# MinJunKang/DualPixelFace

Measured on AMD Instinct MI355X. Metric: train samples/sec, StereoDPNet 1024x1536 DP pair, higher is better.
Workload: dtype f32

## Files before the change

### dualpixelface_amd/csrc/conv_api.hip

```cpp
#include "conv_internal.h"
#include <cstdlib>

namespace {

int g_operand_bf16 = 0;
int g_f32_x9 = -1;
int g_h3_guard = 1;

int clamp_x9(int v) { return v < 0 ? 0 : (v > 2 ? 2 : v); }

int out_dim(int I, int k, int s, int p, int d) { return (I + 2 * p - (d * (k - 1) + 1)) / s + 1; }

DpfConvDesc forward_desc(int N, int C, int ID, int IH, int IW, int K, int kd, int kh, int kw, int sd, int sh, int sw, int pd, int ph, int pw, int dd,
                         int dh, int dw) {
  return {N, C, K, K, 0, ID, IH, IW, out_dim(ID, kd, sd, pd, dd), out_dim(IH, kh, sh, ph, dh), out_dim(IW, kw, sw, pw, dw),
          kd, kh, kw, sd, sh, sw, pd, ph, pw, dd, dh, dw,  0,  K, C,  0,  0};
}
DpfConvDesc transposed_desc(int N, int C, int ID, int IH, int IW, int K, int Ktot, int OD, int OH, int OW, int kd, int kh, int kw, int sd, int sh,
                            int sw, int pd, int ph, int pw, int dd, int dh, int dw, int accumulate) {
  return {N, C, K, Ktot, 0, ID, IH, IW, OD, OH, OW, kd, kh, kw, sd, sh, sw, pd, ph, pw, dd, dh, dw,  1, C, Ktot,  1, accumulate};
}

bool bad_args(const void* a, const void* b, const void* c, int N, int C, int K) { return !a || !b || !c || N <= 0 || C <= 0 || K <= 0; }

int conv_dispatch(const float* x, const float* w, const float* bias, float* out, float* ws, const DpfConvDesc& d, DpfConvStats* stats, hipStream_t st) {
  const int T = d.kd * d.kh * d.kw;
  const bool plain = !stats && !d.accumulate;
  if (!plain && d.K > 128) return DPF_ERR_UNSUPPORTED;
  if (T > DPF_CONV_MAXT)
    return !stats && dpf_wide_eligible(T, d.kd, d.kh, d.kw, d.sd, d.sh, d.sw, d.pd, d.dd, d.dh, d.dw) ? dpf_wide_conv(x, w, bias, out, d, st)
                                                                                                        : DPF_ERR_UNSUPPORTED;
  if (T < 1) return DPF_ERR_UNSUPPORTED;
  for (int k0 = 0; k0 < d.K; k0 += 128) {
    DpfConvDesc s = d;
    s.k0 = k0;
    s.K = d.K - k0 < 128 ? d.K - k0 : 128;
    int rc = DPF_ERR_UNSUPPORTED;
    if (plain && T == 1) rc = dpf_pointwise_conv(x, w, bias, out, s, st);
    if (rc == DPF_ERR_UNSUPPORTED) rc = dpf_igemm2_conv(x, w, bias, out, ws, s, st, stats);
    if (rc == DPF_ERR_UNSUPPORTED && plain) rc = dpf_gen1_conv(x, w, bias, out, ws, s, st);
    if (rc != DPF_OK) return rc;
  }
  return DPF_OK;
}

int wgrad_dispatch(const float* g, const float* x, float* dw, float* ws, long long ws_floats, const DpfWgradDesc& d, int accumulate, hipStream_t st) {
  const int T = d.kd * d.kh * d.kw;
  for (int k0 = 0; k0 < d.K; k0 += 128) {
    DpfWgradDesc s = d;
    s.k0 = k0;
    s.K = d.K - k0 < 128 ? d.K - k0 : 128;
    float* dwk = dw + (long long)k0 * d.C * T;
    int rc = DPF_ERR_UNSUPPORTED;
    if (ws && T == 1) rc = dpf_pointwise_wgrad(g, x, dwk, ws, ws_floats, s, accumulate, st);
    if (rc == DPF_ERR_UNSUPPORTED && ws && T > DPF_CONV_MAXT) rc = dpf_wide_wgrad(g, x, dwk, ws, ws_floats, s, accumulate, st);
    if (rc == DPF_ERR_UNSUPPORTED && ws) rc = dpf_wgrad2(g, x, dwk, ws, ws_floats, s, accumulate, st);
    if (rc == DPF_ERR_UNSUPPORTED) {
      if (!accumulate && hipMemsetAsync(dwk, 0, sizeof(float) * (size_t)s.K * d.C * T, st) != hipSuccess) return DPF_ERR_LAUNCH;
      rc = dpf_gen1_wgrad(g, x, dwk, s, st);
    }
    if (rc != DPF_OK) return rc;
  }
  return DPF_OK;
}

}

const ConvEnv& conv_env() {
  static const ConvEnv env = [] {
    auto num = [](const char* v, int unset) { return v ? atoi(v) : unset; };
    ConvEnv e;
    e.f32_x9 = clamp_x9(num(getenv("DPF_F32_X9"), 2));
    e.igemm2 = num(getenv("DPF_IGEMM2"), 1);
    e.igemm2_tr2 = num(getenv("DPF_IGEMM2_TR2"), 1);
    e.igemm2_1x1 = num(getenv("DPF_IGEMM2_1x1"), 1);
    e.igemm3 = num(getenv("DPF_IGEMM3"), 1);
    e.igemm3_cc = num(getenv("DPF_IGEMM3_CC"), 0);
    e.igemm3_sh = num(getenv("DPF_IGEMM3_SH"), -1);
    e.igemm3_rstep = num(getenv("DPF_IGEMM3_RSTEP"), 1);
    e.igemm3_bf = num(getenv("DPF_IGEMM3_BF"), 1);
    e.g2_pz = num(getenv("DPF_G2_PZ"), 0);
    e.g2_vec_store = num(getenv("DPF_G2_VEC_STORE"), 1);
    e.wgrad2 = num(getenv("DPF_WGRAD2"), 1);
    e.w2_sw1 = num(getenv("DPF_W2_SW1"), 1);
    e.w2_rstep = num(getenv("DPF_W2_RSTEP"), 1);
    e.pointwise = num(getenv("DPF_POINTWISE"), 1);
    return e;
  }();
  return env;
}

int dpf_conv_operand_bf16() { return g_operand_bf16; }
int dpf_conv_f32_x9() { return g_f32_x9 < 0 ? conv_env().f32_x9 : g_f32_x9; }
int dpf_h3_range_guard() { return g_h3_guard; }

extern "C" {

int dpf_set_conv_operand_precision(int bf16) {
  g_operand_bf16 = bf16 ? 1 : 0;
  return DPF_OK;
}
int dpf_get_conv_operand_precision(void) { return g_operand_bf16; }
int dpf_set_f32_matrix_path(int split_bf16) {
  g_f32_x9 = clamp_x9(split_bf16);
  return DPF_OK;
}
int dpf_get_f32_matrix_path(void) { return dpf_conv_f32_x9(); }
int dpf_debug_set_range_guard(int on) {
  g_h3_guard = on ? 1 : 0;
  return DPF_OK;
}

long long dpf_conv_workspace_floats(int T, int reduce, int outc) {
  const long long a = (long long)T * reduce * (((outc + 31) / 32) * 32), b = dpf_igemm2_workspace_floats(T, reduce, outc);
  return a > b ? a : b;
}

int dpf_conv_forward(const float* x, const float* w, const float* bias, float* out, float* ws, int N, int C, int ID, int IH, int IW,
                     int K, int kd, int kh, int kw, int sd, int sh, int sw, int pd, int ph, int pw, int dd, int dh, int dw,
                     void* stream) {
  dpf_clear_error();
  if (bad_args(x, w, out, N, C, K) || !ws) return DPF_ERR_INVALID_ARG;
  const DpfConvDesc d = forward_desc(N, C, ID, IH, IW, K, kd, kh, kw, sd, sh, sw, pd, ph, pw, dd, dh, dw);
  if (d.OD <= 0 || d.OH <= 0 || d.OW <= 0) return DPF_ERR_INVALID_ARG;
  return conv_dispatch(x, w, bias, out, ws, d, nullptr, (hipStream_t)stream);
}

long long dpf_conv_stats_slab_doubles(int N, int K, int OD, int OH, int OW) {
  return 2LL * K * ((long long)N * OD * dpf_div_up(OH, 8) * dpf_div_up(OW, 32) + 64);
// ... 41 lines not shown
```

### dualpixelface_amd/csrc/conv_igemm2.hip

```cpp
#include "conv_internal.h"
#include <type_traits>

namespace {

constexpr int MAXT = 27;
constexpr int NLD = 8;
constexpr int ZPAGE = 16;

struct G2P {
  int N, C, K, Ktot, k0;
  int ID, IH, IW, OD, OH, OW;
  int sxd, sxh, sxw;
  int e0d, e0h, e0w;
  int ext_d, ext_h;
  int pz, thp, thp_shift, odt;
  int planeStride;
  int RS, SR;
  int colshift;
  int rpc, chanStride;
  int nseg;
  int nwseg;
  int T;
  int tilesH, tilesW;
  int ntiles, cpx;
// ... 344 lines not shown
        for (int cp = 0; cp < CC / 2; ++cp)
  #pragma unroll
          for (int m = 0; m < MT; ++m)
  #pragma unroll
            for (int t = 0; t < NT; ++t) acc[m][t] = __builtin_amdgcn_mfma_f32_32x32x2f32(a[cp][m], bb[cp][t], acc[m][t], 0, 0, 0);
      };
      auto touch = [&](const float (&a)[CC / 2][MT], const float (&bb)[CC / 2][NT]) {
  #pragma unroll
        for (int cp = 0; cp < CC / 2; ++cp) {
  #pragma unroll
          for (int m = 0; m < MT; ++m) asm volatile("" ::"v"(a[cp][m]));
  #pragma unroll
          for (int t = 0; t < NT; ++t) asm volatile("" ::"v"(bb[cp][t]));
        }
        asm volatile("" ::: "memory");
      };
      load_ops(aA, bA);
      for (int slot = 0; slot + 1 < nv; slot += 2) {
        touch(aA, bA);
        load_ops(aB, bB);
        __builtin_amdgcn_sched_barrier(6);
        mfmas(aA, bA);
        __builtin_amdgcn_sched_barrier(0);
        touch(aB, bB);
        load_ops(aA, bA);
        __builtin_amdgcn_sched_barrier(6);
        mfmas(aB, bB);
        __builtin_amdgcn_sched_barrier(0);
      }
      if (nv & 1) mfmas(aA, bA);
    }
    __builtin_amdgcn_sched_barrier(0);
    __syncthreads();
    if (single && chunk + 1 < p.nchunks) {
      issue(chunk + 1, 0);
      __syncthreads();
    }
  }

  g2_epilogue<MT, NT>(acc, p, bias, out, smem, tile_id, n, qd, q0h, q0w, wave, l31, hh, tid);
}



typedef unsigned u32x4 __attribute__((ext_vector_type(4)));
typedef __bf16 bf16x8 __attribute__((ext_vector_type(8)));
typedef _Float16 f16x8 __attribute__((ext_vector_type(8)));

__device__ __forceinline__ void split_pair(float x, float y, unsigned& h, unsigned& m, unsigned& l) { dpf_split_pair(x, y, h, m, l); }

constexpr int X9_FIRST = DPF_X9_FIRST;
constexpr int X9_NP = 9 - X9_FIRST;

template <int CC, int NC> struct X9 {
  static constexpr int NU = CC == 4 ? 2 : 1;
  static constexpr int PB = 2 * NC * CC;
  static constexpr int TPG = 16 / CC;
  static constexpr int PD = PB / 4;
};

#ifdef DPF_STAMPS
__device__ unsigned long long g_x9_passes[4];
__device__ unsigned long long g_x9_stamps[8 * 16384];
#define X9_STAMP(slot, val) if (tid == 0 && blockIdx.x < 16384) g_x9_stamps[blockIdx.x * 8 + (slot)] = (val);
#define X9_COUNT(slot) if (tid == 0) atomicAdd(&g_x9_passes[slot], 1ull);
#else
#define X9_STAMP(slot, val)
#define X9_COUNT(slot)
#endif

template <int MT, int NT, int CC, bool SH, int NC = 3>
__global__ __launch_bounds__(256, 2) void igemm3_x9_kernel(const float* __restrict__ x, const unsigned short* __restrict__ wpk,
                                                           const float* __restrict__ bias, float* __restrict__ out, G2P p) {
  extern __shared__ __attribute__((aligned(16))) float smem[];
  static_assert(NT == 2 || NT == 4, "position rows are processed in pairs");
  constexpr int KT = 32 * MT;
  constexpr int NU = X9<CC, NC>::NU, PB = X9<CC, NC>::PB, TPG = X9<CC, NC>::TPG, PD = X9<CC, NC>::PD;
  constexpr int NPROD = NC == 3 ? X9_NP : (NC == 2 ? 3 : 1);
  constexpr int SPV = NC == 3 ? 9 : (NC == 2 ? 6 : 1);
  constexpr int NPS = NT / 2;
  constexpr int NSL = NU * 4;
  const int tid = threadIdx.x;
  const int lane = tid & 63;
  const int wave = __builtin_amdgcn_readfirstlane(tid >> 6);
  const int l31 = lane & 31;
  const int hh = lane >> 5;

  int b = (blockIdx.x & 7) * p.cpx + (blockIdx.x >> 3);
  if (b >= p.ntiles) return;
  X9_STAMP(0, __builtin_readcyclecounter()) X9_STAMP(4, __builtin_amdgcn_s_memrealtime())
  const int tile_id = b;
  const int qd = (b % p.odt) * p.pz; b /= p.odt;
  const int tw = b % p.tilesW; b /= p.tilesW;
  const int th = b % p.tilesH;
  const int n = b / p.tilesH;
  const int q0h = (th / p.rstep) * (p.thp * p.rstep) + th % p.rstep, q0w = tw * 32;
  const int i0d = qd + p.e0d, i0h = q0h + p.e0h;
  const int a0 = q0w + p.e0w - p.colshift;

  const int TG = (p.T + TPG - 1) / TPG;
  const int patchBytes = PB * p.rpc * p.RS;
  const int wBytes = TG * NC * MT * 1024;
  char* s_patch = reinterpret_cast<char*>(smem);
  char* s_w = s_patch + patchBytes;
  int* s_tab = reinterpret_cast<int*>(s_w + (SH ? 2 : 1) * wBytes);
  int* s_red = s_tab + 32;
  int Ex = DPF_H3_EMIN;
  int Erun = DPF_H3_EMIN;
  float scx = 0.f;
  unsigned tbC = 0, tbN = 0;
  unsigned kminL = 0xffffffffu;
  const long long x_chan = (long long)p.ID * p.IH * p.IW;
  const float* xn = x + (long long)n * p.C * x_chan;
  const int nunits = p.rpc * p.SR;

  if (tid < 32) s_tab[tid] = tid < 28 ? PB * p.tapoff[tid] : 0;

  int goff[NU], loff[NU];
#pragma unroll
  for (int j = 0; j < NU; ++j) {
    const unsigned f = tid + 256 * j;
    const unsigned row = (f * p.mSR) >> 20;
    const int seg = f - row * p.SR;
    const unsigned pl = (row * p.mEH) >> 20;
    const int rr = row - pl * p.ext_h;
    const int id = i0d + (int)pl, ih = i0h + rr * p.rstep, iw = a0 + 4 * seg;
    const bool ok = (int)f < nunits && id >= 0 && id < p.ID && ih >= 0 && ih < p.IH && iw >= 0 && iw < p.IW;
    goff[j] = ok ? (int)(((long long)id * p.IH + ih) * p.IW + iw) : -1;
    loff[j] = (int)f < nunits ? PB * ((int)row * p.RS + 4 * seg) : -1;
  }

  f32x4 pv[NU][CC];
  unsigned sp[NU][4][PD];
  auto prefetch = [&](int chunk) {
    const float* xc = xn + (long long)chunk * CC * x_chan;
    const int crem = p.C - chunk * CC;
#pragma unroll
    for (int j = 0; j < NU; ++j)
#pragma unroll
      for (int ch = 0; ch < CC; ++ch) {
        f32x4 v = {0.f, 0.f, 0.f, 0.f};
        if (goff[j] >= 0 && ch < crem) v = *reinterpret_cast<const f32x4*>(xc + (long long)ch * x_chan + goff[j]);
        pv[j][ch] = v;
      }
  };
  auto issue_w = [&](int chunk, int buf) {
    const char* wc = reinterpret_cast<const char*>(wpk) + (long long)chunk * wBytes;
    char* dst = s_w + buf * wBytes;
    const int nws = wBytes >> 4;
    for (int f0 = wave * 64; f0 < nws; f0 += 256) {
      const int f = f0 + lane;
      if (f < nws) glds16(reinterpret_cast<const float*>(wc + f * 16), reinterpret_cast<float*>(dst + f0 * 16));
    }
  };
  auto split_slice = [&](int sl) {
    const int j = sl >> 2, ps = sl & 3;
#pragma unroll
    for (int k = 0; k < CC / 2; ++k) {
      if constexpr (NC == 3) split_pair(pv[j][2 * k][ps], pv[j][2 * k + 1][ps], sp[j][ps][k], sp[j][ps][CC / 2 + k], sp[j][ps][CC + k]);
      else if constexpr (NC == 2) dpf_split_pair_h(pv[j][2 * k][ps] * scx, pv[j][2 * k + 1][ps] * scx, sp[j][ps][k], sp[j][ps][CC / 2 + k]);
      else sp[j][ps][k] = pk_bf16(pv[j][2 * k][ps], pv[j][2 * k + 1][ps]);
    }
  };
  auto pos_max = [&](int j, int ps) {
    float mp = __builtin_fabsf(pv[j][0][ps]);
#pragma unroll
    for (int ch = 1; ch < CC; ++ch) mp = __builtin_fmaxf(mp, __builtin_fabsf(pv[j][ch][ps]));
    return mp;
  };
  auto post_exp = [&]() {
    float pm[NU][4];
#pragma unroll
    for (int j = 0; j < NU; ++j) {
#pragma unroll
      for (int ps = 0; ps < 4; ++ps) pm[j][ps] = __builtin_fmaxf(__builtin_fabsf(pv[j][0][ps]), __builtin_fabsf(pv[j][1][ps]));
#pragma unroll
      for (int ch = 2; ch < CC; ch += 2)
#pragma unroll
        for (int ps = 0; ps < 4; ++ps) pm[j][ps] = __builtin_fmaxf(__builtin_fmaxf(pm[j][ps], __builtin_fabsf(pv[j][ch][ps])), __builtin_fabsf(pv[j][ch + 1][ps]));
    }
    float m = 0.f;
    kminL = 0xffffffffu;
// ... 14 lines not shown
    return e > 254 ? 254 : (e < DPF_H3_EMIN ? DPF_H3_EMIN : e);
  };
  auto tb_of = [&](int e) {
    return (unsigned)(e < 1 ? 1 : (e > 254 ? 254 : e)) << 23;
  };
  int Enext = Ex;
  auto next_chunk_scale = [&]() {
    const int e = read_exp();
    Erun = e > Erun ? e : Erun;
    const int lo = Erun - DPF_H3_MAXDROP;
    Enext = (e > Ex || (e < Ex - 3 && e > DPF_H3_EMIN)) ? (e > lo ? e : lo) : Ex;
    scx = dpf_h3_scale(Enext);
    tbN = p.guard ? tb_of(Enext - DPF_H3_RANGE) : 0u;
  };
  auto next_residual_scale = [&](int pass_next) {
    const int e = read_exp();
    const int lo = Erun - DPF_H3_MAXDROP;
    const int en = Ex + e - 141;
    Enext = en > lo ? en : lo;
    if (Enext > Ex) Enext = Ex;
    scx = __builtin_bit_cast(float, (unsigned)(127 + Ex - Enext) << 23);
    tbN = pass_next < DPF_H3_MAXPASS ? tb_of(Enext - DPF_H3_RANGE + 141 - Ex) : 0u;
  };
  auto lane_defers = [&](int par) {
    const bool fl = tbN != 0u && kminL < tbN - 1u;
    if (fl) s_red[8 + par] = 1;
    return __builtin_amdgcn_ballot_w64(fl) != 0ull;
  };
  auto split_masked = [&]() {
#pragma unroll
    for (int j = 0; j < NU; ++j)
#pragma unroll
      for (int ps = 0; ps < 4; ++ps) {
        const float ml = __builtin_bit_cast(unsigned, pos_max(j, ps)) >= tbN ? scx : 0.f;
#pragma unroll
        for (int k = 0; k < CC / 2; ++k) dpf_split_pair_h(pv[j][2 * k][ps] * ml, pv[j][2 * k + 1][ps] * ml, sp[j][ps][k], sp[j][ps][CC / 2 + k]);
      }
  };
  auto residual_update = [&]() {
#pragma unroll
    for (int j = 0; j < NU; ++j)
#pragma unroll
      for (int ps = 0; ps < 4; ++ps) {
        const float ml = __builtin_bit_cast(unsigned, pos_max(j, ps)) >= tbC ? 0.f : scx;
#pragma unroll
        for (int ch = 0; ch < CC; ++ch) pv[j][ch][ps] *= ml;
      }
  };
  auto store_split = [&]() {
#pragma unroll
    for (int j = 0; j < NU; ++j)
      if (loff[j] >= 0) {
        u32x4* dst = reinterpret_cast<u32x4*>(s_patch + loff[j]);
#pragma unroll
        for (int i = 0; i < PD; ++i) {
          const int e = 4 * i;
          const u32x4 v = {sp[j][e / PD][e % PD], sp[j][(e + 1) / PD][(e + 1) % PD], sp[j][(e + 2) / PD][(e + 2) % PD], sp[j][(e + 3) / PD][(e + 3) % PD]};
          dst[i] = v;
        }
      }
  };

  f32x16 acc[MT][NT];
#pragma unroll
  for (int m = 0; m < MT; ++m)
#pragma unroll
    for (int t = 0; t < NT; ++t)
#pragma unroll
      for (int j = 0; j < 16; ++j) acc[m][t][j] = 0.f;
  auto rescale_acc = [&](int de) {
#pragma unroll
    for (int m = 0; m < MT; ++m)
#pragma unroll
      for (int t = 0; t < NT; ++t)
#pragma unroll
        for (int j = 0; j < 16; ++j) acc[m][t][j] = __builtin_ldexpf(acc[m][t][j], de);
  };

  int lb[NT];
#pragma unroll
  for (int t = 0; t < NT; ++t) {
    const int r = wave * NT + t, rz = r >> p.thp_shift, ry = r & (p.thp - 1);
    lb[t] = PB * (rz * p.planeStride + ry * p.RS + l31 + p.colshift);
  }

  if constexpr (NC == 2) {
    if (tid < 2) s_red[8 + tid] = 0;
  }
  if constexpr (SH) issue_w(0, 0);
  prefetch(0);
  int par = 0;
  if constexpr (SH) {
    bool wdef = false;
    if constexpr (NC == 2) {
      post_exp();
      __syncthreads();
      next_chunk_scale();
      Ex = Enext;
      wdef = lane_defers(par);
    }
#pragma unroll
    for (int sl = 0; sl < NSL; ++sl) split_slice(sl);
    if constexpr (NC == 2) {
      if (__builtin_expect(wdef, 0)) split_masked();
    }
  }

  int pass = 0;
  for (int chunk = 0; chunk < p.nchunks;) {
    if constexpr (!SH) {
      bool wdef = false;
      if (pass == 0) issue_w(chunk, 0);
      if constexpr (NC == 2) {
        post_exp();
        __syncthreads();
        if (pass == 0) next_chunk_scale(); else next_residual_scale(pass);
        wdef = lane_defers(par);
      }
#pragma unroll
      for (int sl = 0; sl < NSL; ++sl) split_slice(sl);
      if constexpr (NC == 2) {
        if (__builtin_expect(wdef, 0)) split_masked();
      }
    }
    bool more = false;
    int dflag = 0;
    if constexpr (NC == 2) {
      if constexpr (SH) {
        if (chunk > 0 || pass > 0) dflag = s_red[8 + par];
      }
      if (tid == 0) s_red[8 + (par ^ 1)] = 0;
      if (__builtin_expect(Enext != Ex, 0)) { rescale_acc(Ex - Enext); Ex = Enext; X9_COUNT(2) }
      X9_COUNT(0)
      if (pass > 0) { X9_COUNT(1) }
      tbC = tbN;
    }
// ... 526 lines not shown
}

__global__ void igemm2_pack_bf16_kernel(const float* __restrict__ w, unsigned short* __restrict__ wpk, int wA, int wB, int T, int KT, int nchunks,
                                        int mode, int k0, int K, int C) {
  const long long total = (long long)nchunks * T * 8 * KT + 2 * ZPAGE;
  for (long long i = (long long)blockIdx.x * blockDim.x + threadIdx.x; i < total; i += (long long)gridDim.x * blockDim.x) {
    float v = 0.f;
    if (i >= 2 * ZPAGE) {
      const long long e = i - 2 * ZPAGE;
      const int ii = (int)(e & 3);
      const int k = (int)((e >> 2) % KT);
      const int half = (int)((e / (4LL * KT)) & 1);
      const int t = (int)((e / (8LL * KT)) % T);
      const int chunk = (int)(e / (8LL * KT * T));
      const int c = chunk * 8 + half * 4 + ii;
      if (k < K && c < C) {
        const int a = mode == 0 ? k0 + k : c;
        const int bb = mode == 0 ? c : k0 + k;
        v = w[((long long)a * wB + bb) * T + t];
      }
    }
    wpk[i] = (unsigned short)(pk_bf16(v, 0.f) & 0xffffu);
  }
}

unsigned magic20(int d) { return (unsigned)(((1u << 20) + d - 1) / d); }

template <typename W, typename P>
struct TileLaunch {
  const float* x; const W* wpk; const float* bias; float* out; const P& p; size_t lds; long long blocks; hipStream_t st;
};

template <int MT, int NT, int CC, bool BF = false>
int launch_g2(const TileLaunch<float, G2P>& a) {
  return conv_launch<igemm2_kernel<MT, NT, CC, BF>>(dim3((unsigned)a.blocks), dim3(256), a.lds, a.st, a.x, a.wpk, a.bias, a.out, a.p);
}
template <int MT, int NT, int CC>
int launch_x9(bool sh, int NC, const TileLaunch<unsigned short, G2P>& a) {
  const dim3 grid((unsigned)a.blocks), block(256);
  switch (2 * NC + (sh ? 1 : 0)) {
    case 7: return conv_launch<igemm3_x9_kernel<MT, NT, CC, true, 3>>(grid, block, a.lds, a.st, a.x, a.wpk, a.bias, a.out, a.p);
    case 6: return conv_launch<igemm3_x9_kernel<MT, NT, CC, false, 3>>(grid, block, a.lds, a.st, a.x, a.wpk, a.bias, a.out, a.p);
    case 5: return conv_launch<igemm3_x9_kernel<MT, NT, CC, true, 2>>(grid, block, a.lds, a.st, a.x, a.wpk, a.bias, a.out, a.p);
    case 4: return conv_launch<igemm3_x9_kernel<MT, NT, CC, false, 2>>(grid, block, a.lds, a.st, a.x, a.wpk, a.bias, a.out, a.p);
    case 3: return conv_launch<igemm3_x9_kernel<MT, NT, CC, true, 1>>(grid, block, a.lds, a.st, a.x, a.wpk, a.bias, a.out, a.p);
    default: return conv_launch<igemm3_x9_kernel<MT, NT, CC, false, 1>>(grid, block, a.lds, a.st, a.x, a.wpk, a.bias, a.out, a.p);
  }
}
template <int CC, bool BF = false>
int launch_t2(const TileLaunch<float, T2P>& a) {
  return conv_launch<igemm2_tr2_kernel<CC, BF>>(dim3((unsigned)a.blocks), dim3(256), a.lds, a.st, a.x, a.wpk, a.bias, a.out, a.p);
}

int launch_x9(int MT, int NT, int CC9, bool sh, int NC, const TileLaunch<unsigned short, G2P>& a) {
  if (CC9 == 4) {
    if (MT == 1) return NT == 4 ? launch_x9<1, 4, 4>(sh, NC, a) : launch_x9<1, 2, 4>(sh, NC, a);
    return launch_x9<2, 2, 4>(sh, NC, a);
  }
  if (MT == 1) return NT == 4 ? launch_x9<1, 4, 8>(sh, NC, a) : launch_x9<1, 2, 8>(sh, NC, a);
  return launch_x9<2, 2, 8>(sh, NC, a);
}

int x9_try(const float* x, const float* w, const float* bias, float* out, float* ws, const DpfConvDesc& d, const G2P& p, int k_off, int kn, int NT,
           DpfConvStats* stats, hipStream_t st, int NC, int mt_fit = 0) {
  const ConvEnv& env = conv_env();
  constexpr int x9_min_c = 8;
  const int T = d.kd * d.kh * d.kw, MT = (kn + 31) / 32, TH = 4 * NT;
  if (!env.igemm3 || (NC >= 2 && !dpf_conv_f32_x9()) || MT > 2 || NT * MT > 4 || d.C < x9_min_c) return DPF_ERR_UNSUPPORTED;
  G2P q = p;
  q.K = kn; q.k0 = d.k0 + k_off;
  q.rstep = (env.igemm3_rstep && d.kd == 1 && d.kh > 1 && d.dh > 1) ? d.dh : 1;
  const int dhl = d.dh / q.rstep;
  int CC9 = ((T + 1) / 2) * 2 < ((T + 3) / 4) * 4 ? 8 : 4;
  if (env.igemm3_cc == 4 || env.igemm3_cc == 8) CC9 = env.igemm3_cc;
  const int NU9 = CC9 == 4 ? 2 : 1, PB9 = 2 * NC * CC9;
  auto set_pz = [&](int pz) {
    q.pz = pz; q.thp = TH / pz; q.thp_shift = 0;
    while ((1 << q.thp_shift) < q.thp) ++q.thp_shift;
    q.odt = dpf_div_up(d.OD, pz);
    q.ext_d = (pz - 1) + (d.kd - 1) * d.dd + 1;
    q.ext_h = (q.thp - 1) + (d.kh - 1) * dhl + 1;
    q.planeStride = q.ext_h * q.RS; q.SR = q.RS / 4; q.rpc = q.ext_d * q.ext_h;
    return q.rpc * q.SR;
  };
  const int TG = (T + 16 / CC9 - 1) / (16 / CC9);
  int best = 0, best_units = 1 << 30, sh = 0;
  for (int shc : {1, 0}) {
    if (best || (env.igemm3_sh >= 0 && shc != env.igemm3_sh)) continue;
    for (int pz : {1, 2, 4}) {
      if (!(pz == 1 || (d.kd > 1 && pz <= TH / 2 && pz <= d.OD))) continue;
      const int units = set_pz(pz);
      const size_t l9 = (size_t)PB9 * q.rpc * q.RS + (size_t)(shc ? 2 : 1) * TG * NC * (mt_fit > MT ? mt_fit : MT) * 1024 + 256;
      if (units <= NU9 * 256 && 2 * l9 <= 160 * 1024 && units < best_units) { best = pz; best_units = units; sh = shc; }
    }
  }
  if (!best || TG < 2) return DPF_ERR_UNSUPPORTED;
  set_pz(best);
  const size_t lds9 = (size_t)PB9 * q.rpc * q.RS + (size_t)(sh ? 2 : 1) * TG * NC * MT * 1024 + 256;
  if ((long long)NU9 * 256 * (q.SR > q.ext_h ? q.SR : q.ext_h) >= (1LL << 20)) return DPF_ERR_UNSUPPORTED;
  const int sgn = d.transposed ? -1 : 1;
  const int t0 = d.transposed ? ((d.kd - 1) * d.dd * q.ext_h + (d.kh - 1) * dhl) * q.RS + (d.kw - 1) * d.dw : 0;
  for (int u = 0; u < 28; ++u) {
    const int c = u % d.kw, b2 = (u / d.kw) % d.kh, a = u / (d.kw * d.kh);
    q.tapoff[u] = u < T ? t0 + sgn * ((a * d.dd * q.ext_h + b2 * dhl) * q.RS + c * d.dw) : 0;
  }
  q.nchunks = (d.C + CC9 - 1) / CC9;
  q.tilesH = dpf_div_up(d.OH, q.thp * q.rstep) * q.rstep;
  q.tilesW = dpf_div_up(d.OW, 32);
  q.mSR = magic20(q.SR); q.mEH = magic20(q.ext_h);
  const long long nt9 = (long long)d.N * q.odt * q.tilesH * q.tilesW;
  if (nt9 <= 0 || nt9 > 0x3fffffffLL) return DPF_ERR_INVALID_ARG;
  q.ntiles = (int)nt9;
  q.cpx = (int)((nt9 + 7) / 8);
  q.stats = nullptr;
  if (stats) {
    if (nt9 * d.K * 2 > stats->capacity_doubles) return DPF_ERR_UNSUPPORTED;
    if (k_off > 0 && stats->parts != (int)nt9) return DPF_ERR_LAUNCH;
    q.stats = stats->slab; q.statsK = d.K; q.statsk0 = k_off;
  }
  unsigned short* wp = reinterpret_cast<unsigned short*>(ws);
  const long long total = (long long)q.nchunks * TG * MT * 512;
  int* wexp = reinterpret_cast<int*>(wp + ((total * NC + 7) & ~7LL));
  q.wexp = wexp;
  q.guard = dpf_h3_range_guard();
  if (NC == 2)
    hipLaunchKernelGGL(igemm3_pack_x9h_kernel, dim3(32 * MT), dim3(256), 0, st, w, wp, d.wA, d.wB, T, TG, MT, CC9, q.nchunks, d.mode, q.k0, kn, d.C, wexp);
  else
    hipLaunchKernelGGL(igemm3_pack_x9_kernel, dim3(dpf_ew_grid(total)), dim3(256), 0, st, w, wp, d.wA, d.wB, T, TG, MT, CC9, NC, q.nchunks, d.mode, q.k0, kn,
                       d.C);
  if (dpf_check_launch() != DPF_OK) return DPF_ERR_LAUNCH;
  if (stats) stats->parts = (int)nt9;
  return launch_x9(MT, NT, CC9, sh != 0, NC, {x, wp, bias, out, q, lds9, 8LL * q.cpx, st});
}

int igemm2_tr2(const float* x, const float* w, const float* bias, float* out, float* ws, const DpfConvDesc& d, hipStream_t st) {
  if (!conv_env().igemm2_tr2) return DPF_ERR_UNSUPPORTED;
  if (d.kd != 3 || d.kh != 3 || d.kw != 3 || d.sd != 2 || d.sh != 2 || d.sw != 2 || d.pd != 1 || d.ph != 1 || d.pw != 1 || d.dd != 1 ||
      d.dh != 1 || d.dw != 1)
    return DPF_ERR_UNSUPPORTED;
  if (d.OD > 2 * d.ID || d.OH > 2 * d.IH || d.OW > 2 * d.IW) return DPF_ERR_UNSUPPORTED;
  const long long x_chan = (long long)d.ID * d.IH * d.IW;
  if (9 * x_chan >= (1LL << 30)) return DPF_ERR_UNSUPPORTED;
  const bool bf = dpf_conv_operand_bf16() != 0;
  const int CC = 8;
  T2P p{};
  p.N = d.N; p.C = d.C; p.Ktot = d.Ktot;
  p.ID = d.ID; p.IH = d.IH; p.IW = d.IW; p.OD = d.OD; p.OH = d.OH; p.OW = d.OW;
  p.RS = 36; p.SR = 9; p.rpc = 2 * 5; p.chanStride = p.rpc * p.RS;
  p.nseg = CC * p.rpc * p.SR;
  p.nwseg = bf ? 27 * 32 : 27 * CC * 32 / 4;
  p.nchunks = (d.C + CC - 1) / CC;
  p.QD = dpf_div_up(d.OD, 2);
  p.tilesH = dpf_div_up(dpf_div_up(d.OH, 2), 4);
  p.tilesW = dpf_div_up(dpf_div_up(d.OW, 2), 32);
  const long long ntiles = (long long)d.N * p.QD * p.tilesH * p.tilesW;
  if (ntiles <= 0 || ntiles > 0x3fffffffLL) return DPF_ERR_INVALID_ARG;
  p.ntiles = (int)ntiles;
  p.cpx = (int)((ntiles + 7) / 8);
  p.mSR = magic20(p.SR); p.mRPC = magic20(p.rpc); p.mEH = magic20(5);
  p.vec = conv_env().g2_vec_store;
  const size_t lds = 2 * (size_t)(CC * p.chanStride + 4 * p.nwseg) * sizeof(float);
  for (int k0 = 0; k0 < d.K; k0 += 32) {
    const int Kc = d.K - k0 < 32 ? d.K - k0 : 32;
    p.K = Kc; p.k0 = d.k0 + k0;
    const long long total = (long long)p.nchunks * 27 * CC * 32 + ZPAGE;
    if (bf)
      hipLaunchKernelGGL(igemm2_pack_bf16_kernel, dim3(dpf_ew_grid(total)), dim3(256), 0, st, w, reinterpret_cast<unsigned short*>(ws), d.wA, d.wB, 27,
                         32, p.nchunks, d.mode, p.k0, Kc, d.C);
    else
      hipLaunchKernelGGL(igemm2_pack_kernel, dim3(dpf_ew_grid(total)), dim3(256), 0, st, w, ws, d.wA, d.wB, 27, 32, CC, p.nchunks, d.mode, p.k0, Kc, d.C);
    if (dpf_check_launch() != DPF_OK) return DPF_ERR_LAUNCH;
    const TileLaunch<float, T2P> a{x, ws, bias, out, p, lds, 8LL * p.cpx, st};
    int rc;
    if (bf) rc = launch_t2<8, true>(a);
    else switch (CC) { case 2: rc = launch_t2<2>(a); break; case 4: rc = launch_t2<4>(a); break; default: rc = launch_t2<8>(a); break; }
    if (rc != DPF_OK) return rc;
  }
  return DPF_OK;
}

struct G2Plan {
  G2P p;
  int T, MT, KT;
  int NT;
  int single;
// ... 54 lines not shown
  p.accum = d.accumulate;
  p.rstep = 1;
  p.vec = conv_env().g2_vec_store && (d.OW & 3) == 0 && (reinterpret_cast<uintptr_t>(out) & 15) == 0;
  if (!d.transposed) {
    p.sxd = d.sd; p.sxh = d.sh; p.sxw = d.sw;
    p.e0d = -d.pd; p.e0h = -d.ph; p.e0w = -d.pw;
  } else {
    p.sxd = p.sxh = p.sxw = 1;
    p.e0d = d.pd - (d.kd - 1) * d.dd; p.e0h = d.ph - (d.kh - 1) * d.dh; p.e0w = d.pw - (d.kw - 1) * d.dw;
  }
  const int ext_w = 31 * p.sxw + (d.kw - 1) * d.dw + 1;
  p.colshift = ((p.e0w % 4) + 4) % 4;
  p.RS = ((p.colshift + ext_w + 3) / 4) * 4;
  const int pz_over = conv_env().g2_pz;
  auto pz_ok = [&](int pz) { return pz == 1 || (d.kd > 1 && pz <= TH / 2 && pz <= d.OD); };
  auto pz_cost = [&](int pz) {
    const int thp = TH / pz;
    return (double)((pz - 1) * p.sxd + (d.kd - 1) * d.dd + 1) * ((thp - 1) * p.sxh + (d.kh - 1) * d.dh + 1) / (double)(pz * thp);
  };
  p.pz = 1;
  for (int pz : {2, 4})
    if (pz_ok(pz) && pz_cost(pz) < pz_cost(p.pz) - 1e-9) p.pz = pz;
  if ((pz_over == 1 || pz_over == 2 || pz_over == 4) && pz_ok(pz_over)) p.pz = pz_over;
  p.thp = TH / p.pz;
  p.thp_shift = 0;
  while ((1 << p.thp_shift) < p.thp) ++p.thp_shift;
  p.odt = dpf_div_up(d.OD, p.pz);
  p.ext_d = (p.pz - 1) * p.sxd + (d.kd - 1) * d.dd + 1;
  p.ext_h = (p.thp - 1) * p.sxh + (d.kh - 1) * d.dh + 1;
  p.planeStride = p.ext_h * p.RS;
  p.SR = p.RS / 4;
  p.rpc = p.ext_d * p.ext_h;
  p.chanStride = p.rpc * p.RS;
}

void g2_tap_steps(const DpfConvDesc& d, G2P& p) {
  const int sgn = d.transposed ? -1 : 1;
  const int stepA = sgn * d.dd * p.ext_h * p.RS, stepB = sgn * d.dh * p.RS;
  p.stepC = sgn * d.dw;
  p.incB = stepB - (d.kw - 1) * p.stepC;
  p.incA = stepA - (d.kh - 1) * stepB - (d.kw - 1) * p.stepC;
  p.steps = 0;
  for (int t = 0; t < p.T; ++t) {
    const int c = t % d.kw, b = (t / d.kw) % d.kh;
    const unsigned long long code = t == p.T - 1 ? 3 : (c + 1 < d.kw ? 0 : (b + 1 < d.kh ? 1 : 2));
    p.steps |= code << (2 * t);
  }
  p.tap0 = d.transposed ? ((d.kd - 1) * d.dd * p.ext_h + (d.kh - 1) * d.dh) * p.RS + (d.kw - 1) * d.dw : 0;
}

int g2_x9_route(const float* x, const float* w, const float* bias, float* out, float* ws, const DpfConvDesc& d, const G2Plan& g, DpfConvStats* stats,
                hipStream_t st) {
  const G2P& p = g.p;
  if (!(g.T > 4 && p.sxd == 1 && p.sxh == 1 && p.sxw == 1 && (!g.bf_mode || (conv_env().igemm3_bf && !(d.K > 64 && d.kd == 1)))))
    return DPF_ERR_UNSUPPORTED;
  const int nc = g.bf_mode ? 1 : dpf_conv_f32_nc();
  if (d.K <= 64) return x9_try(x, w, bias, out, ws, d, p, 0, d.K, g.MT == 1 ? 4 : 2, stats, st, nc);
  for (int k_off = 0; k_off < d.K; k_off += 64) {
    const int rc = x9_try(x, w, bias, out, ws, d, p, k_off, d.K - k_off < 64 ? d.K - k_off : 64, 2, stats, st, nc, 2);
    if (rc == DPF_ERR_UNSUPPORTED && k_off == 0) return rc;
    if (rc != DPF_OK) return rc == DPF_ERR_UNSUPPORTED ? DPF_ERR_LAUNCH : rc;
  }
  return DPF_OK;
}

size_t g2_buf_bytes(const G2Plan& g, int cc) { return (size_t)(cc * g.p.chanStride + g.T * cc * g.KT) * sizeof(float); }
size_t g2_bf_buf_bytes(const G2Plan& g) { return (size_t)8 * g.p.chanStride * sizeof(float) + (size_t)g.T * g.KT * 16; }

bool g2_chunk(const DpfConvDesc& d, G2Plan& g) {
  constexpr int lds_target = 53 * 1024;
  const G2P& p = g.p;
  auto nseg_of = [&](int cc) { return cc * p.rpc * p.SR; };
  auto fits = [&](int cc) { return 2 * g2_buf_bytes(g, cc) <= (size_t)lds_target && nseg_of(cc) <= NLD * 256; };
  const long long ntiles_est = (long long)d.N * p.odt * dpf_div_up(d.OH, p.thp) * dpf_div_up(d.OW, 32);
  g.CC = g.bf ? 8 : (ntiles_est >= 512 && fits(2)) ? 2 : fits(8) ? 8 : fits(4) ? 4 : 2;
  return g.bf ? (nseg_of(8) <= 2 * NLD * 256 && 2 * g2_bf_buf_bytes(g) <= 160 * 1024)
              : (nseg_of(g.CC) <= NLD * 256 && 2 * g2_buf_bytes(g, g.CC) <= 160 * 1024);
}

int launch_g2(int MT, int NT, int CC, bool bf, const TileLaunch<float, G2P>& a) {
  if (bf) {
    if (NT == 4) return MT == 1 ? launch_g2<1, 4, 8, true>(a) : launch_g2<2, 4, 8, true>(a);
    switch (MT) {
      case 1: return launch_g2<1, 2, 8, true>(a);
      case 2: return launch_g2<2, 2, 8, true>(a);
      case 3: return launch_g2<3, 2, 8, true>(a);
      default: return launch_g2<4, 2, 8, true>(a);
    }
  }
  const int cc = CC == 8 ? 0 : (CC == 4 ? 1 : 2);
  switch ((NT == 4 ? (MT == 1 ? 0 : 1) : (MT < 4 ? MT + 1 : 5)) * 3 + cc) {
    case 0: return launch_g2<1, 4, 8>(a);
    case 1: return launch_g2<1, 4, 4>(a);
    case 2: return launch_g2<1, 4, 2>(a);
    case 3: return launch_g2<2, 4, 8>(a);
    case 4: return launch_g2<2, 4, 4>(a);
    case 5: return launch_g2<2, 4, 2>(a);
    case 6: return launch_g2<1, 2, 8>(a);
    case 7: return launch_g2<1, 2, 4>(a);
    case 8: return launch_g2<1, 2, 2>(a);
    case 9: return launch_g2<2, 2, 8>(a);
    case 10: return launch_g2<2, 2, 4>(a);
    case 11: return launch_g2<2, 2, 2>(a);
    case 12: return launch_g2<3, 2, 8>(a);
    case 13: return launch_g2<3, 2, 4>(a);
    case 14: return launch_g2<3, 2, 2>(a);
    case 15: return launch_g2<4, 2, 8>(a);
    case 16: return launch_g2<4, 2, 4>(a);
// ... 77 lines not shown
```

### dualpixelface_amd/csrc/conv_internal.h

```cpp
#pragma once
#include "dpf_common.h"

struct DpfConvDesc {
  int N, C, K, Ktot, k0;
  int ID, IH, IW, OD, OH, OW;
  int kd, kh, kw, sd, sh, sw, pd, ph, pw, dd, dh, dw;
  int transposed;
  int wA, wB, mode;
  int accumulate;
};

struct ConvEnv {
  int f32_x9;
  int igemm2;
  int igemm2_tr2;
  int igemm2_1x1;
  int igemm3;
  int igemm3_cc;
  int igemm3_sh;
  int igemm3_rstep;
  int igemm3_bf;
  int g2_pz;
  int g2_vec_store;
  int wgrad2;
  int w2_sw1;
  int w2_rstep;
  int pointwise;
};
const ConvEnv& conv_env();

constexpr int DPF_CONV_MAXT = 27;

int dpf_conv_operand_bf16();
int dpf_conv_f32_x9();
int dpf_h3_range_guard();
inline int dpf_conv_f32_nc() { return dpf_conv_f32_x9() == 2 ? 2 : 3; }

#ifdef __HIPCC__
template <auto Kern, typename... A>
int conv_launch(dim3 grid, dim3 block, size_t lds, hipStream_t st, A... args) {
  static size_t granted = 48 * 1024;
  if (lds > granted) {
    if (hipFuncSetAttribute((const void*)Kern, hipFuncAttributeMaxDynamicSharedMemorySize, (int)lds) != hipSuccess) return DPF_ERR_LAUNCH;
    granted = lds;
  }
  hipLaunchKernelGGL(Kern, grid, block, lds, st, args...);
  return dpf_check_launch();
}
#endif

struct DpfConvStats {
  double* slab;
  long long capacity_doubles;
  int parts;
};
int dpf_igemm2_conv(const float* x, const float* w, const float* bias, float* out, float* ws, const DpfConvDesc& d, hipStream_t st,
                    DpfConvStats* stats = nullptr);
long long dpf_igemm2_workspace_floats(int T, int reduce, int outc);
int dpf_gen1_conv(const float* x, const float* w, const float* bias, float* out, float* ws, const DpfConvDesc& d, hipStream_t st);

struct DpfWgradDesc {
  int N, C, K, Ktot, k0;
  int ID, IH, IW, QD, QH, QW;
  int kd, kh, kw, sd, sh, sw, pd, ph, pw, dd, dh, dw;
};
int dpf_wgrad2(const float* g, const float* x, float* dw, float* ws, long long ws_floats, const DpfWgradDesc& d, int accumulate, hipStream_t st);
long long dpf_wgrad2_workspace_floats(int T, int C, int K);
int dpf_gen1_wgrad(const float* g, const float* x, float* dw, const DpfWgradDesc& d, hipStream_t st);

int dpf_pointwise_conv(const float* x, const float* w, const float* bias, float* out, const DpfConvDesc& d, hipStream_t st);
int dpf_pointwise_wgrad(const float* g, const float* x, float* dw, float* ws, long long ws_floats, const DpfWgradDesc& d, int accumulate,
                        hipStream_t st);
long long dpf_pointwise_wgrad_workspace_floats(int C, int K);

// ... 75 lines not shown
```

Baseline: 27.49.

## Route stride-2 f32 convolutions through the split-precision igemm3 x9 kernel

```diff
diff --git a/dualpixelface_amd/csrc/conv_api.hip b/dualpixelface_amd/csrc/conv_api.hip
--- a/dualpixelface_amd/csrc/conv_api.hip
+++ b/dualpixelface_amd/csrc/conv_api.hip
@@ -75,6 +75,7 @@
     e.igemm2_tr2 = num(getenv("DPF_IGEMM2_TR2"), 1);
     e.igemm2_1x1 = num(getenv("DPF_IGEMM2_1x1"), 1);
     e.igemm3 = num(getenv("DPF_IGEMM3"), 1);
+    e.igemm3_s2 = e.igemm3 != 2;
     e.igemm3_cc = num(getenv("DPF_IGEMM3_CC"), 0);
     e.igemm3_sh = num(getenv("DPF_IGEMM3_SH"), -1);
     e.igemm3_rstep = num(getenv("DPF_IGEMM3_RSTEP"), 1);
diff --git a/dualpixelface_amd/csrc/conv_igemm2.hip b/dualpixelface_amd/csrc/conv_igemm2.hip
--- a/dualpixelface_amd/csrc/conv_igemm2.hip
+++ b/dualpixelface_amd/csrc/conv_igemm2.hip
@@ -420,6 +420,7 @@
 constexpr int X9_FIRST = DPF_X9_FIRST;
 constexpr int X9_NP = 9 - X9_FIRST;
 
+constexpr int X9_S2_NU = 3;
 template <int CC, int NC> struct X9 {
   static constexpr int NU = CC == 4 ? 2 : 1;
   static constexpr int PB = 2 * NC * CC;
@@ -437,13 +438,14 @@
 #define X9_COUNT(slot)
 #endif
 
-template <int MT, int NT, int CC, bool SH, int NC = 3>
+template <int MT, int NT, int CC, bool SH, int NC = 3, bool S2 = false>
 __global__ __launch_bounds__(256, 2) void igemm3_x9_kernel(const float* __restrict__ x, const unsigned short* __restrict__ wpk,
                                                            const float* __restrict__ bias, float* __restrict__ out, G2P p) {
   extern __shared__ __attribute__((aligned(16))) float smem[];
   static_assert(NT == 2 || NT == 4, "position rows are processed in pairs");
   constexpr int KT = 32 * MT;
-  constexpr int NU = X9<CC, NC>::NU, PB = X9<CC, NC>::PB, TPG = X9<CC, NC>::TPG, PD = X9<CC, NC>::PD;
+  static_assert(!S2 || (CC == 4 && NC == 2), "the stride-2 staging is built for 16-byte position records");
+  constexpr int NU = S2 ? X9_S2_NU : X9<CC, NC>::NU, PB = X9<CC, NC>::PB, TPG = X9<CC, NC>::TPG, PD = X9<CC, NC>::PD;
   constexpr int NPROD = NC == 3 ? X9_NP : (NC == 2 ? 3 : 1);
   constexpr int SPV = NC == 3 ? 9 : (NC == 2 ? 6 : 1);
   constexpr int NPS = NT / 2;
@@ -463,8 +465,8 @@
   const int th = b % p.tilesH;
   const int n = b / p.tilesH;
   const int q0h = (th / p.rstep) * (p.thp * p.rstep) + th % p.rstep, q0w = tw * 32;
-  const int i0d = qd + p.e0d, i0h = q0h + p.e0h;
-  const int a0 = q0w + p.e0w - p.colshift;
+  const int i0d = (S2 ? qd * p.sxd : qd) + p.e0d, i0h = (S2 ? q0h * p.sxh : q0h) + p.e0h;
+  const int a0 = (S2 ? 2 * q0w : q0w) + p.e0w - p.colshift;
 
   const int TG = (p.T + TPG - 1) / TPG;
   const int patchBytes = PB * p.rpc * p.RS;
@@ -495,7 +497,7 @@
     const int id = i0d + (int)pl, ih = i0h + rr * p.rstep, iw = a0 + 4 * seg;
     const bool ok = (int)f < nunits && id >= 0 && id < p.ID && ih >= 0 && ih < p.IH && iw >= 0 && iw < p.IW;
     goff[j] = ok ? (int)(((long long)id * p.IH + ih) * p.IW + iw) : -1;
-    loff[j] = (int)f < nunits ? PB * ((int)row * p.RS + 4 * seg) : -1;
+    loff[j] = (int)f < nunits ? PB * ((int)row * p.RS + (S2 ? 2 : 4) * seg) : -1;
   }
 
   f32x4 pv[NU][CC];
@@ -616,6 +618,15 @@
     for (int j = 0; j < NU; ++j)
       if (loff[j] >= 0) {
         u32x4* dst = reinterpret_cast<u32x4*>(s_patch + loff[j]);
+        if constexpr (S2) {
+          u32x4* dso = reinterpret_cast<u32x4*>(s_patch + loff[j] + PB * (p.RS >> 1));
+#pragma unroll
+          for (int ps = 0; ps < 4; ++ps) {
+            const u32x4 v = {sp[j][ps][0], sp[j][ps][1], sp[j][ps][2], sp[j][ps][3]};
+            ((ps & 1) ? dso : dst)[ps >> 1] = v;
+          }
+          continue;
+        }
 #pragma unroll
         for (int i = 0; i < PD; ++i) {
           const int e = 4 * i;
@@ -645,7 +656,7 @@
 #pragma unroll
   for (int t = 0; t < NT; ++t) {
     const int r = wave * NT + t, rz = r >> p.thp_shift, ry = r & (p.thp - 1);
-    lb[t] = PB * (rz * p.planeStride + ry * p.RS + l31 + p.colshift);
+    lb[t] = S2 ? PB * (rz * p.sxd * p.planeStride + ry * p.sxh * p.RS + l31) : PB * (rz * p.planeStride + ry * p.RS + l31 + p.colshift);
   }
 
   if constexpr (NC == 2) {
@@ -1278,6 +1289,12 @@
   return conv_launch<igemm2_tr2_kernel<CC, BF>>(dim3((unsigned)a.blocks), dim3(256), a.lds, a.st, a.x, a.wpk, a.bias, a.out, a.p);
 }
 
+template <int MT>
+int launch_x9_s2(const TileLaunch<unsigned short, G2P>& a) {
+  const dim3 grid((unsigned)a.blocks), block(256);
+  return conv_launch<igemm3_x9_kernel<MT, 2, 4, false, 2, true>>(grid, block, a.lds, a.st, a.x, a.wpk, a.bias, a.out, a.p);
+}
+
 int launch_x9(int MT, int NT, int CC9, bool sh, int NC, const TileLaunch<unsigned short, G2P>& a) {
   if (CC9 == 4) {
     if (MT == 1) return NT == 4 ? launch_x9<1, 4, 4>(sh, NC, a) : launch_x9<1, 2, 4>(sh, NC, a);
@@ -1291,28 +1308,32 @@
            DpfConvStats* stats, hipStream_t st, int NC, int mt_fit = 0) {
   const ConvEnv& env = conv_env();
   constexpr int x9_min_c = 8;
+  const bool s2 = p.sxw == 2;
+  if (s2) NT = 2;
   const int T = d.kd * d.kh * d.kw, MT = (kn + 31) / 32, TH = 4 * NT;
+  if (s2 && (NC != 2 || env.igemm3_cc == 8)) return DPF_ERR_UNSUPPORTED;
   if (!env.igemm3 || (NC >= 2 && !dpf_conv_f32_x9()) || MT > 2 || NT * MT > 4 || d.C < x9_min_c) return DPF_ERR_UNSUPPORTED;
   G2P q = p;
   q.K = kn; q.k0 = d.k0 + k_off;
-  q.rstep = (env.igemm3_rstep && d.kd == 1 && d.kh > 1 && d.dh > 1) ? d.dh : 1;
+  q.rstep = (env.igemm3_rstep && d.kd == 1 && d.kh > 1 && d.dh > 1 && !s2) ? d.dh : 1;
   const int dhl = d.dh / q.rstep;
   int CC9 = ((T + 1) / 2) * 2 < ((T + 3) / 4) * 4 ? 8 : 4;
   if (env.igemm3_cc == 4 || env.igemm3_cc == 8) CC9 = env.igemm3_cc;
-  const int NU9 = CC9 == 4 ? 2 : 1, PB9 = 2 * NC * CC9;
+  if (s2) CC9 = 4;
+  const int NU9 = s2 ? X9_S2_NU : (CC9 == 4 ? 2 : 1), PB9 = 2 * NC * CC9;
   auto set_pz = [&](int pz) {
     q.pz = pz; q.thp = TH / pz; q.thp_shift = 0;
     while ((1 << q.thp_shift) < q.thp) ++q.thp_shift;
     q.odt = dpf_div_up(d.OD, pz);
-    q.ext_d = (pz - 1) + (d.kd - 1) * d.dd + 1;
-    q.ext_h = (q.thp - 1) + (d.kh - 1) * dhl + 1;
+    q.ext_d = (pz - 1) * p.sxd + (d.kd - 1) * d.dd + 1;
+    q.ext_h = (q.thp - 1) * p.sxh + (d.kh - 1) * dhl + 1;
     q.planeStride = q.ext_h * q.RS; q.SR = q.RS / 4; q.rpc = q.ext_d * q.ext_h;
     return q.rpc * q.SR;
   };
   const int TG = (T + 16 / CC9 - 1) / (16 / CC9);
   int best = 0, best_units = 1 << 30, sh = 0;
   for (int shc : {1, 0}) {
-    if (best || (env.igemm3_sh >= 0 && shc != env.igemm3_sh)) continue;
+    if (best || (s2 ? shc != 0 : (env.igemm3_sh >= 0 && shc != env.igemm3_sh))) continue;
     for (int pz : {1, 2, 4}) {
       if (!(pz == 1 || (d.kd > 1 && pz <= TH / 2 && pz <= d.OD))) continue;
       const int units = set_pz(pz);
@@ -1329,6 +1350,10 @@
   for (int u = 0; u < 28; ++u) {
     const int c = u % d.kw, b2 = (u / d.kw) % d.kh, a = u / (d.kw * d.kh);
     q.tapoff[u] = u < T ? t0 + sgn * ((a * d.dd * q.ext_h + b2 * dhl) * q.RS + c * d.dw) : 0;
+    if (s2 && u < T) {
+      const int col = q.colshift + c * d.dw;
+      q.tapoff[u] = (a * d.dd * q.ext_h + b2 * dhl) * q.RS + (col & 1) * (q.RS / 2) + col / 2;
+    }
   }
   q.nchunks = (d.C + CC9 - 1) / CC9;
   q.tilesH = dpf_div_up(d.OH, q.thp * q.rstep) * q.rstep;
@@ -1356,7 +1381,9 @@
                        d.C);
   if (dpf_check_launch() != DPF_OK) return DPF_ERR_LAUNCH;
   if (stats) stats->parts = (int)nt9;
-  return launch_x9(MT, NT, CC9, sh != 0, NC, {x, wp, bias, out, q, lds9, 8LL * q.cpx, st});
+  const TileLaunch<unsigned short, G2P> a{x, wp, bias, out, q, lds9, 8LL * q.cpx, st};
+  if (s2) return MT == 1 ? launch_x9_s2<1>(a) : launch_x9_s2<2>(a);
+  return launch_x9(MT, NT, CC9, sh != 0, NC, a);
 }
 
 int igemm2_tr2(const float* x, const float* w, const float* bias, float* out, float* ws, const DpfConvDesc& d, hipStream_t st) {
@@ -1517,8 +1544,9 @@
 int g2_x9_route(const float* x, const float* w, const float* bias, float* out, float* ws, const DpfConvDesc& d, const G2Plan& g, DpfConvStats* stats,
                 hipStream_t st) {
   const G2P& p = g.p;
-  if (!(g.T > 4 && p.sxd == 1 && p.sxh == 1 && p.sxw == 1 && (!g.bf_mode || (conv_env().igemm3_bf && !(d.K > 64 && d.kd == 1)))))
-    return DPF_ERR_UNSUPPORTED;
+  const bool s1 = p.sxd == 1 && p.sxh == 1 && p.sxw == 1;
+  const bool s2 = !d.transposed && conv_env().igemm3_s2 && p.sxw == 2 && p.sxh == 2 && (p.sxd == 1 || p.sxd == 2) && !g.bf_mode && dpf_conv_f32_x9() == 2;
+  if (!(g.T > 4 && (s1 || s2) && (!g.bf_mode || (conv_env().igemm3_bf && !(d.K > 64 && d.kd == 1))))) return DPF_ERR_UNSUPPORTED;
   const int nc = g.bf_mode ? 1 : dpf_conv_f32_nc();
   if (d.K <= 64) return x9_try(x, w, bias, out, ws, d, p, 0, d.K, g.MT == 1 ? 4 : 2, stats, st, nc);
   for (int k_off = 0; k_off < d.K; k_off += 64) {
diff --git a/dualpixelface_amd/csrc/conv_internal.h b/dualpixelface_amd/csrc/conv_internal.h
--- a/dualpixelface_amd/csrc/conv_internal.h
+++ b/dualpixelface_amd/csrc/conv_internal.h
@@ -20,6 +20,7 @@
   int igemm3_sh;
   int igemm3_rstep;
   int igemm3_bf;
+  int igemm3_s2;
   int g2_pz;
   int g2_vec_store;
   int wgrad2;
```

Result: no change. 27.64 (median of 6 runs) (+0.5%).
